# laughtervv/DISN

Hardware: AMD Instinct MI355X
Metric: SDF point queries/sec (137x137 img, 2048-pt batch, VGG-16 encode + two-stream query per batch) (higher is better)
Workload: dtype f32 results (products: two-term f16 split on v_mfma_f32_32x32x16_f16, ~22-bit operands, fp32 accumulate; gather / projection / resize / fc: fp32 FMA)

## Files before the change

### disn_amd/_lib.py

```python
from __future__ import annotations

import ctypes as C
import os
from typing import Optional

HERE = os.path.dirname(os.path.abspath(__file__))
LIB_PATH = os.environ.get("DISN_AMD_LIB") or os.path.join(HERE, "csrc", "libdisn_amd.so")
ABI_VERSION = 10

c_float_p = C.c_void_p


class DisnLibraryError(RuntimeError):
    pass


class DisnError(RuntimeError):
    def __init__(self, fn: str, status: int):
        kind = {-1: "invalid argument", -2: "unsupported shape", -3: "workspace too small",
                -4: "did not converge"}.get(
            status, "hipError_t %d" % status if status > 0 else "error")
        super().__init__("%s failed: %s (status %d)" % (fn, kind, status))
        self.status = status

# ... 51 lines not shown


I, Z, P, F, L = C.c_int, C.c_size_t, C.c_void_p, C.c_float, C.c_int64
SIGNATURES = {
    "disn_abi_version": (I, []),
    "disn_pack_kn": (I, [P, I, I, I, P, P]),
    "disn_pack_kn_x3_bytes": (Z, [I, I]),
    "disn_pack_kn_x3": (I, [P, I, I, P, P]),
    "disn_conv3x3_x3_workspace_bytes": (Z, [I, I, I, I, I]),
    "disn_conv3x3_x3": (I, [P, I, I, I, I, P, P, I, I, P, P, Z, P]),
    "disn_pack_conv_h2_bytes": (Z, [I, I]),
    "disn_pack_conv_h2": (I, [P, I, I, P, P]),
    "disn_conv_h2_gain_span": (I, [P, I, I, P, P]),
    "disn_conv1_1_workspace_bytes": (Z, []),
    "disn_conv1_1": (I, [P, I, I, I, P, P, I, P, P, P, Z, P]),
    "disn_conv3x3_h2_workspace_bytes": (Z, [I]),
    "disn_conv3x3_h2": (I, [P, I, I, I, I, P, P, I, I, P, P, P, I, P, Z, P]),
    "disn_conv3x3_h2_plan": (I, [I, I, I, I, I, I, P, P]),
    "disn_resize_bilinear": (I, [P, I, I, I, I, P, I, I, I, I, P]),
    "disn_vgg16_workspace_bytes": (Z, [I]),
    "disn_vgg16_forward": (I, [C.POINTER(VggWeights), P, I, P, C.POINTER(C.c_void_p * 5), P, P, Z, P]),
    "disn_vgg16_conv_stack": (I, [C.POINTER(VggWeights), P, I, P, C.POINTER(C.c_void_p * 5), P, P, Z, P]),
    "disn_conv3x3_workspace_bytes": (Z, [I, I, I, I, I]),
    "disn_conv3x3": (I, [P, I, I, I, I, P, P, I, I, P, P, Z, P]),
    "disn_conv3x3_planned_workspace_bytes": (Z, [I, I, I, I, I, I, I, I]),
    "disn_conv3x3_planned": (I, [P, I, I, I, I, P, P, I, I, P, P, Z, I, I, I, P]),
    "disn_maxpool2x2": (I, [P, I, I, I, I, P, P]),
    "disn_fc_workspace_bytes": (Z, [I, I, I]),
    "disn_fc": (I, [P, I, I, P, P, I, I, P, P, Z, P]),
    "disn_pack_dense_h2_bytes": (Z, [I, I]),
# ... 146 lines not shown
```

### disn_amd/csrc/api.hip

```cpp
#include "../../include/disn_amd.h"

#include "kernels.hpp"
#include "mesh_bvh.hpp"
#include "tuning.hpp"

#include <new>

using namespace disn;

#define DISN_TRY(expr)                    \
  do {                                    \
    hipError_t _e = (expr);               \
    if (_e != hipSuccess) return (int)_e; \
  } while (0)
#define DISN_RC(expr)        \
  do {                       \
    const int _rc = (expr);  \
    if (_rc) return _rc;     \
  } while (0)

namespace {

struct Bump {
  char* base;
// ... 522 lines not shown
  for (int i = 0; i < 3; ++i)
    if (!w->fc_w[i] || !w->fc_b[i]) return false;
  return true;
}

bool vgg_all_h2(const disn_vgg_weights_t* w) {
  for (int i = 0; i < 13; ++i)
    if (!w->conv_w_h2[i]) return false;
  return true;
}

int vgg_features(const disn_vgg_weights_t* w, const float* img, int B, float* resized,
                 float* const taps[5], float* featmap, const VggWs& s, const float** xio,
                 hipStream_t st, int i0 = 0, int i1 = 13) {
  const bool h2 = vgg_all_h2(w);
  if (i0 == 0)
    DISN_TRY(resize_bilinear_launch(img, B, DISN_IMG_H, DISN_IMG_W, 3, resized, DISN_VGG_SIZE,
                                    DISN_VGG_SIZE, 3, 0, st, 0, h2 ? s.amax : nullptr, h2 ? 14 * B * 64 : 0));
  const float* x = i0 == 0 ? resized : *xio;
  bool toggle = false;
  const size_t gws_cap = (size_t)((char*)s.fc_ws - (char*)s.gemm_ws);
  for (int i = 0; i < i1; ++i) {
    const VggLayer& L = kVgg[i];
    float* out = L.tap >= 0 ? taps[L.tap] : (L.hw >= 112 ? s.bufA : (toggle ? s.bufB : s.bufA));
    if (L.tap < 0 && L.hw < 112) toggle = !toggle;
    if (kPoolAfter[i]) toggle = false;
    if (i < i0) continue;
    bool pooled = false;
    if (h2 && i == 0) {
      DISN_TRY(conv1_1_direct_launch(x, B, L.hw, L.hw, static_cast<const float*>(w->conv_w_h2[0]), w->conv_b[0], 1, out,
                                     s.amax + (size_t)B * 64, st, 64));
    } else if (h2) {
      DISN_TRY(conv_h2_launch(x, B, L.hw, L.hw, L.cin, w->conv_w_h2[i], w->conv_b[i], L.cout, 1,
                              s.amax + (size_t)B * 64 * i, out, kPoolAfter[i] ? s.bufP : nullptr,
                              s.amax + (size_t)B * 64 * (i + 1), st, w->strict_forms == 1 ? kConvTilingStrict : kConvTilingAuto, 64));
      pooled = kPoolAfter[i];
    } else {
      DISN_RC(conv3x3_impl(x, B, L.hw, L.hw, L.cin, w->conv_w[i], w->conv_b[i], L.cout, 1, out, s.gemm_ws, gws_cap, st,
                           w->conv_w_x3[i], kPoolAfter[i] ? s.bufP : nullptr, &pooled));
    }
    x = out;
    if (L.tap >= 0 && featmap)
      DISN_TRY(resize_bilinear_launch(taps[L.tap], B, kTap[L.tap].hw, kTap[L.tap].hw, kTap[L.tap].ch,
                                      featmap, DISN_IMG_H, DISN_IMG_W, DISN_FEAT_DIM,
// ... 401 lines not shown
                      const float* pts_rot, int B, int N, float* resized224, float* const taps[5],
                      float* embedding, float* featmap, float* sdf, void* ws, size_t ws_bytes,
                      void* stream) {
  if (!ctx || !vgg_weights_ok(vw) || !mlp_weights_ok(mw) || !img || !trans_mat || !pts || !pts_rot ||
      !taps_ok(taps) || !embedding || !sdf || !ws || B <= 0 || N <= 0)
    return DISN_E_ARG;
  if ((long)B * N > kChunk || vw->num_classes != DISN_EMBED_DIM) return DISN_E_SHAPE;
  hipStream_t st = (hipStream_t)stream;
  const EncQueryWs e = encq_layout(ws, B, N, vw->num_classes);
  if (e.total > ws_bytes) return DISN_E_WS;
  float* resized = resized224 ? resized224 : e.vgg.resized;
  if (ctx->pipe_wait) DISN_TRY(hipStreamWaitEvent(st, ctx->pipe_wait, 0));
  const EncPlan p = encq_plan(vw, mw, B, N, featmap != nullptr);
  switch (p.form) {
    case ENC_FUSED_SMALL:
      return encq_fused_small(ctx, vw, mw, img, trans_mat, pts, pts_rot, B, N, resized, taps, embedding, sdf, e, st);
    case ENC_DENSE_H2:
      return encq_dense_h2(ctx, vw, mw, img, trans_mat, pts, pts_rot, B, N, resized, taps, embedding, featmap, sdf,
                           p.hb, p.strict, e, st);
    default:
      return encq_gemm_chain(ctx, vw, mw, img, trans_mat, pts, pts_rot, B, N, resized, taps, embedding, featmap, sdf,
                             e, st);
  }
}

int disn_build_featmap(const float* const taps[5], int B, float* featmap, void* stream) {
  if (!taps_ok(taps) || !featmap || B <= 0) return DISN_E_ARG;
  for (int i = 0; i < 5; ++i)
    DISN_TRY(resize_bilinear_launch(taps[i], B, kTap[i].hw, kTap[i].hw, kTap[i].ch, featmap, DISN_IMG_H,
                                    DISN_IMG_W, DISN_FEAT_DIM, kTap[i].off, (hipStream_t)stream));
  return 0;
// ... 643 lines not shown
```

### disn_amd/csrc/conv_h2.hip

```cpp
#include "kernels.hpp"
#include "tuning.hpp"
#include "h2_common.hpp"

#include <type_traits>

namespace disn {


__device__ __forceinline__ void h2_colmax_chunk(const float* __restrict__ p, long base, int mid, int inner,
                                                float* __restrict__ cmax_inner, float* __restrict__ cmax_mid,
                                                unsigned* tab_i, unsigned* tab_m) {
  const bool big_i = inner > 1024, big_m = mid > 1024;
  for (int i = threadIdx.x; i < 1024; i += 256) { tab_i[i] = 0u; tab_m[i] = 0u; }
  __syncthreads();
#pragma unroll
  for (int k = 0; k < 4; ++k) {
    const long e = base + (long)(k * 256 + threadIdx.x) * 4;
    const float4 v = *reinterpret_cast<const float4*>(p + e);
    const float a[4] = {fabsf(v.x), fabsf(v.y), fabsf(v.z), fabsf(v.w)};
    if (cmax_inner) {
      const int c0 = (int)(e % inner);
#pragma unroll
      for (int q = 0; q < 4; ++q) {
        if (big_i) atomicMax(reinterpret_cast<unsigned*>(cmax_inner) + c0 + q, __float_as_uint(a[q]));
// ... 466 lines not shown
    } else {
#pragma unroll
      for (int mb = 0; mb < MB; ++mb)
#pragma unroll
        for (int e = 0; e < NE; e += 2) {
          float m = fmaxf(val[mb][e], val[mb][e + 1]);
          m = fmaxf(m, __shfl_xor(m, 32));
          const int tx = (L0 & 15) + e0 + e, x = x0 + tx, y = y0 + 2 * mb;
          if (L0 < 16 && tx < TW && y + 1 < H && x + 1 < W) pb[((size_t)(y >> 1) * Wp + (x >> 1)) * Cout] = m;
        }
    }
  }
  CH2_STAMP(14);
}

template <int RT>
__global__ __launch_bounds__(256) void conv1_1_direct_kernel(const float* __restrict__ in, const float* __restrict__ w,
                                                             const float* __restrict__ bias, int B, int H, int W,
                                                             int relu, float* __restrict__ out,
                                                             float* __restrict__ out_amax, int amax_stride) {
  constexpr int PW = 40;
  constexpr int WR = 2 * RT + 2;
  constexpr int WE = WR * 34 * 3;
  constexpr int LQ = (WE + 255) / 256;
  __shared__ __attribute__((aligned(16))) float win[2][WR * 3 * PW];
  __shared__ __attribute__((aligned(16))) float wl[27 * 64];
  __shared__ float red[4];
  const int tid = threadIdx.x, c4 = tid & 15, pg = (tid >> 4) & 7, ry = tid >> 7;
  for (int i = tid; i < 27 * 16; i += 256)
    reinterpret_cast<float4*>(wl)[i] = reinterpret_cast<const float4*>(w)[i];
  __syncthreads();
  float4 wr[27];
#pragma unroll
  for (int k = 0; k < 27; ++k) wr[k] = *reinterpret_cast<const float4*>(&wl[k * 64 + 4 * c4]);
  const float4 bv = *reinterpret_cast<const float4*>(bias + 4 * c4);
  const int segs_x = (W + 31) >> 5, rows2 = (H + 2 * RT - 1) / (2 * RT);
  const long ntile = (long)B * rows2 * segs_x;
  float vmax = 0.f;
  int buf = 0, bcur = -1;
  auto flush = [&](int bimg) {
    float m = vmax;
#pragma unroll
// ... 21 lines not shown
    for (int k = 0; k < LQ; ++k) {
      const int i = tid + 256 * k;
      const int r = i / 102, rem = i - r * 102, px = rem / 3, c = rem - px * 3;
      const int yy = y0 - 1 + r, xx = x0 - 1 + px;
      v[k] = (i < WE && yy >= 0 && yy < H && xx >= 0 && xx < W) ? img[((size_t)yy * W + xx) * 3 + c] : 0.f;
    }
  };
  auto win_store = [&](int bf, const float (&v)[LQ]) {
#pragma unroll
    for (int k = 0; k < LQ; ++k) {
      const int i = tid + 256 * k;
      const int r = i / 102, rem = i - r * 102, px = rem / 3, c = rem - px * 3;
      if (i < WE) win[bf][(r * 3 + c) * PW + px] = v[k];
    }
  };
  float nxt[LQ];
  if ((long)blockIdx.x < ntile) {
    win_load(blockIdx.x, nxt);
    win_store(0, nxt);
  }
  __syncthreads();
  for (long tl = blockIdx.x; tl < ntile; tl += gridDim.x, buf ^= 1) {
    int b, y0, x0;
    tile_of(tl, b, y0, x0);
    if (out_amax && amax_stride && bcur >= 0 && b != bcur) flush(bcur);
    bcur = b;
    const bool more = tl + gridDim.x < ntile;
    if (more) win_load(tl + gridDim.x, nxt);
#pragma unroll 1
    for (int q = 0; q < RT; ++q) {
    float4 a[4] = {bv, bv, bv, bv};
#pragma unroll
    for (int r = 0; r < 3; ++r)
#pragma unroll
      for (int c = 0; c < 3; ++c) {
        const float* pl = &win[buf][((2 * q + ry + r) * 3 + c) * PW + 4 * pg];
        const float4 v0 = *reinterpret_cast<const float4*>(pl);
        const float2 v1 = *reinterpret_cast<const float2*>(pl + 4);
        const float v[6] = {v0.x, v0.y, v0.z, v0.w, v1.x, v1.y};
#pragma unroll
        for (int dx = 0; dx < 3; ++dx) {
          const float4 ww = wr[(r * 3 + dx) * 3 + c];
#pragma unroll
// ... 3 lines not shown
          }
        }
      }
    const int y = y0 + 2 * q + ry;
#pragma unroll
    for (int p = 0; p < 4; ++p) {
      float4 o = a[p];
      if (relu) { o.x = fmaxf(o.x, 0.f); o.y = fmaxf(o.y, 0.f); o.z = fmaxf(o.z, 0.f); o.w = fmaxf(o.w, 0.f); }
      const int x = x0 + 4 * pg + p;
      if (y < H && x < W) {
        *reinterpret_cast<float4*>(out + (((size_t)b * H + y) * W + x) * 64 + 4 * c4) = o;
        vmax = fmaxf(fmaxf(fmaxf(vmax, fabsf(o.x)), fabsf(o.y)), fmaxf(fabsf(o.z), fabsf(o.w)));
      }
    }
    }
    if (more) win_store(buf ^ 1, nxt);
    __syncthreads();
  }
  if (out_amax && bcur >= 0) flush(amax_stride ? bcur : 0);
}

hipError_t conv1_1_direct_launch(const float* in, int B, int H, int W, const float* w_hwio, const float* bias, int relu,
                                 float* out, float* out_amax, hipStream_t st, int amax_stride) {
  const int rt = B >= kConvWideMinImages ? 4 : 1;
  const long ntile = (long)B * ((H + 2 * rt - 1) / (2 * rt)) * ((W + 31) / 32);
  const int grid = (int)(ntile < 512 ? ntile : 512);
  if (rt == 4) hipLaunchKernelGGL(conv1_1_direct_kernel<4>, dim3(grid), dim3(256), 0, st, in, w_hwio, bias, B, H, W, relu, out, out_amax, amax_stride);
  else hipLaunchKernelGGL(conv1_1_direct_kernel<1>, dim3(grid), dim3(256), 0, st, in, w_hwio, bias, B, H, W, relu, out, out_amax, amax_stride);
  return hipGetLastError();
}

bool conv_h2_supported(int H, int W, int Cin, int Cout) {
  return Cin > 0 && Cin % 64 == 0 && Cout > 0 && Cout % 64 == 0 && H > 0 && W > 0 && H < 32768 && W < 32768 &&
         (size_t)H * W * (Cin > Cout ? Cin : Cout) < (size_t)1 << 31;
}

#ifndef CH2_UBENCH
namespace {
long form_grid(int form, int B, int H, int W, int Cout) {
  const ConvFormGeom& g = kConvForms[form];
  return (long)B * ((H + g.th - 1) / g.th) * ((W + g.tw - 1) / g.tw) * (Cout / g.nch);
}

// ... 191 lines not shown
size_t disn_conv1_1_workspace_bytes(void) { return 256; }

int disn_conv1_1(const float* in, int B, int H, int W, const float* w_hwio, const float* bias, int relu, float* out,
                 float* out_amax, void* ws, size_t ws_bytes, void* stream) {
  if (!in || !w_hwio || !bias || !out || !ws || B <= 0 || H <= 0 || W <= 0) return DISN_E_ARG;
  if (ws_bytes < 256) return DISN_E_WS;
  hipStream_t st = (hipStream_t)stream;
  float* slots = static_cast<float*>(ws);
  hipError_t e = hipSuccess;
  if (out_amax) e = hipMemsetAsync(slots, 0, 256, st);
  if (e == hipSuccess) e = disn::conv1_1_direct_launch(in, B, H, W, w_hwio, bias, relu, out, out_amax ? slots : nullptr, st);
  if (e == hipSuccess && out_amax) e = disn::amax_fold_launch(slots, out_amax, st);
  return e == hipSuccess ? 0 : (int)e;
}

}
#endif
```

### disn_amd/csrc/elementwise.hip

```cpp
#include "kernels.hpp"
#include "h2_common.hpp"

namespace disn {

#define DISN_FEAT 1472
#define DISN_FEAT4 368
#define DISN_IMG 137

template <int VEC>
__global__ __launch_bounds__(256) void resize_kernel(const float* __restrict__ in, int B, int Hin,
                                                     int Win, int C, float* __restrict__ out,
                                                     int Hout, int Wout, int out_cstride,
                                                     int out_coff, float sy, float sx,
                                                     float* __restrict__ zero, int nzero) {
  for (size_t i = (size_t)blockIdx.x * blockDim.x + threadIdx.x; i < (size_t)nzero; i += (size_t)gridDim.x * blockDim.x) zero[i] = 0.f;
  const int cv = C / VEC;
  const size_t total = (size_t)B * Hout * Wout * cv;
  for (size_t i = (size_t)blockIdx.x * blockDim.x + threadIdx.x; i < total;
       i += (size_t)gridDim.x * blockDim.x) {
    const int c = (int)(i % cv) * VEC;
    size_t pidx = i / cv;
    const int ox = (int)(pidx % Wout);
    pidx /= Wout;
    const int oy = (int)(pidx % Hout);
    const int b = (int)(pidx / Hout);
    const float fy = (float)oy * sy, fx = (float)ox * sx;
    const int ylo = (int)floorf(fy), xlo = (int)floorf(fx);
    const int yhi = min(ylo + 1, Hin - 1), xhi = min(xlo + 1, Win - 1);
    const float yl = fy - (float)ylo, xl = fx - (float)xlo;
    const float* base = in + (size_t)b * Hin * Win * C + c;
    const float* ptl = base + ((size_t)ylo * Win + xlo) * C;
    const float* ptr = base + ((size_t)ylo * Win + xhi) * C;
    const float* pbl = base + ((size_t)yhi * Win + xlo) * C;
    const float* pbr = base + ((size_t)yhi * Win + xhi) * C;
    float* po = out + ((size_t)(b * Hout + oy) * Wout + ox) * out_cstride + out_coff + c;
    if (VEC == 4) {
      const float4 tl = *reinterpret_cast<const float4*>(ptl);
      const float4 tr = *reinterpret_cast<const float4*>(ptr);
      const float4 bl = *reinterpret_cast<const float4*>(pbl);
      const float4 br = *reinterpret_cast<const float4*>(pbr);
      float4 o;
#define DISN_LERP(f)                              \
  {                                               \
    const float top = tl.f + (tr.f - tl.f) * xl;  \
    const float bot = bl.f + (br.f - bl.f) * xl;  \
    o.f = top + (bot - top) * yl;                 \
  }
      DISN_LERP(x) DISN_LERP(y) DISN_LERP(z) DISN_LERP(w)
#undef DISN_LERP
      *reinterpret_cast<float4*>(po) = o;
    } else {
      const float top = *ptl + (*ptr - *ptl) * xl;
      const float bot = *pbl + (*pbr - *pbl) * xl;
      *po = top + (bot - top) * yl;
    }
  }
}

static inline int grid_for(size_t total, int cap = 8192) {
  size_t b = (total + 255) / 256;
  if (b > (size_t)cap) b = cap;
  if (b < 1) b = 1;
  return (int)b;
}

hipError_t resize_bilinear_launch(const float* in, int B, int Hin, int Win, int C, float* out,
                                  int Hout, int Wout, int out_cstride, int out_coff,
                                  hipStream_t st, int max_blocks, float* zero, int nzero) {
  const int cap = max_blocks > 0 ? max_blocks : 8192;
// ... 742 lines not shown
```

### disn_amd/csrc/h2_common.hpp

```cpp
#pragma once
#include <hip/hip_runtime.h>

#include "kernels.hpp"

namespace disn {

typedef _Float16 ch_h8 __attribute__((ext_vector_type(8)));
typedef _Float16 ch_h4 __attribute__((ext_vector_type(4)));
typedef float ch_f16v __attribute__((ext_vector_type(16)));
typedef float ch_f2v __attribute__((ext_vector_type(2)));

namespace ch2 {
__host__ __device__ inline float pow2_scale(float amax, int target_exp) {
  union { float f; unsigned u; } a;
  a.f = amax;
  const int e = (int)((a.u >> 23) & 0xffu) - 127;
  if (!(amax > 0.f) || e > 100 || e < -100) return 1.0f;
  a.u = (unsigned)(127 + target_exp - e) << 23;
  return a.f;
}
__host__ __device__ constexpr int sigma(int i) {
  return i < 4 ? i : (i < 12 ? i + 12 : (i < 16 ? i - 8 : (i < 20 ? i + 8 : (i < 28 ? i - 12 : i))));
}
__host__ __device__ constexpr int quad_row(int q, int g) {
  return sigma(8 * q + 4 * g);
// ... 107 lines not shown
```

### disn_amd/csrc/kernels.hpp

```cpp
#pragma once
#include <hip/hip_runtime.h>
#include <stddef.h>
#include <stdint.h>

#include "../../include/disn_amd.h"

struct disn_ctx {
  hipStream_t aux;
  hipEvent_t ev[10];
  hipEvent_t pipe_wait = nullptr, pipe_record = nullptr;
};

namespace disn {

#ifdef __HIPCC__
typedef float nt_v4f __attribute__((ext_vector_type(4)));
__device__ __forceinline__ float4 nt_load4(const float* p) {
  const nt_v4f v = __builtin_nontemporal_load(reinterpret_cast<const nt_v4f*>(p));
  return make_float4(v[0], v[1], v[2], v[3]);
}
__device__ __forceinline__ void nt_store4(float* p, const float4& v) {
  nt_v4f t;
  t[0] = v.x; t[1] = v.y; t[2] = v.z; t[3] = v.w;
  __builtin_nontemporal_store(t, reinterpret_cast<nt_v4f*>(p));
// ... 295 lines not shown
  int form;
  int grid, block;
  int tiles_x, tiles_y;
};
ConvPlan conv_h2_plan(int B, int H, int W, int Cin, int Cout, int tiling);
hipError_t conv_h2_launch(const float* in, int B, int H, int W, int Cin, const void* wimg, const float* bias,
                          int Cout, int relu, const float* in_amax, float* out, float* pool_out, float* out_amax,
                          hipStream_t st, int tiling = kConvTilingAuto, int amax_stride = 0);

struct ConvH2Dev;
bool conv_h2w_supported(int H, int W, int Cin, int Cout);
hipError_t conv_h2w_launch(const ConvH2Dev& d, const ConvPlan& plan, hipStream_t st);

hipError_t conv1_1_direct_launch(const float* in, int B, int H, int W, const float* w_hwio, const float* bias, int relu,
                                 float* out, float* out_amax, hipStream_t st, int amax_stride = 0);

struct DenseH2Prob {
  const float* a;
  int lda;
  const float* a2;
  int lda2, k1;
  const float* in_bias;
  int in_bias_rows;
  const unsigned char* wimg;
  int Kimg;
  const float* bias;
  const float* in_amax;
  const float* in_amax2;
  int in_amax2_n;
  float* out;
// ... 57 lines not shown
```

### disn_amd/engine.py

```python
from __future__ import annotations

from dataclasses import dataclass
from typing import Dict, List, Optional

import time

import numpy as np
import torch

from . import ops
from ._lib import MLP_FIELDS, MlpWeights, VggWeights, lib
from .weights import MLP_SCOPES, VGG_CONV_NAMES, WeightStore


class DeviceWeights:

    def __init__(self, store: WeightStore, device: torch.device, conv_h2: bool = True, equalise: bool = True):
        if not store.complete():
            raise ValueError("WeightStore is incomplete")
        self.device = device
        self.num_classes = store.num_classes
        self._keep: List[torch.Tensor] = []
        dev = lambda a: self._hold(torch.from_numpy(np.ascontiguousarray(a, np.float32)).to(device))
        if equalise:
# ... 87 lines not shown
        for f in MLP_FIELDS:
            assert getattr(m, f), f
        self.mlp = m
        torch.cuda.current_stream(device).synchronize()

    def _hold(self, t: torch.Tensor) -> torch.Tensor:
        self._keep.append(t)
        return t


FOLD_MIN_POINTS = 32768


@dataclass
class Encoded:
    resized: torch.Tensor
    taps: List[torch.Tensor]
    embedding: torch.Tensor
    featmap: Optional[torch.Tensor]
    pred: Optional[torch.Tensor] = None
    pmap: Optional[dict] = None
    pmap_amax: Optional[dict] = None
    units: str = "true"


class SdfEngine:

    def __init__(self, store: Optional[WeightStore], device: Optional[torch.device] = None, fused: bool = True,
                 conv_h2: bool = True, weights: Optional[DeviceWeights] = None, equalise: bool = True,
                 strict: bool = False):
        if device is None:
# ... 71 lines not shown
        if enc.pmap is None:
            enc.pmap = {}
        if image_index not in enc.pmap:
            with torch.cuda.device(self.device):
                enc.pmap[image_index] = ops.fold_local(self.weights.mlp, self.featmap_of(enc)[image_index])
        return enc.pmap[image_index]

    def pmap_amax_of(self, enc: Encoded, image_index: int) -> torch.Tensor:
        if enc.pmap_amax is None:
            enc.pmap_amax = {}
        if image_index not in enc.pmap_amax:
            with torch.cuda.device(self.device):
                enc.pmap_amax[image_index] = ops.amax(self.pmap_of(enc, image_index))
        return enc.pmap_amax[image_index]

    def encode_query(self, imgs, pts, trans_mat, pts_rot=None, keep_featmap: bool = False):
        imgs, pts, trans_mat = self._dev(imgs), self._dev(pts), self._dev(trans_mat)
        pts_rot = pts if pts_rot is None else self._dev(pts_rot)
        with torch.cuda.device(self.device):
            ws = self._workspace("encq", lib().disn_encode_query_workspace_bytes(pts.shape[0], pts.shape[1]))
            resized, taps, emb, featmap, sdf = ops.encode_query(self._ctx, self._vgg, self.weights.mlp,
                                                                imgs, trans_mat, pts, pts_rot, ws, keep_featmap)
        return Encoded(resized, taps, emb, featmap, units=self._units()), sdf

    def query(self, enc: Encoded, pts, trans_mat, pts_rot=None, fold: Optional[bool] = None,
              fused: Optional[bool] = None) -> torch.Tensor:
        pts = self._dev(pts)
        pts_rot = pts if pts_rot is None else self._dev(pts_rot)
        trans_mat = self._dev(trans_mat)
        with torch.cuda.device(self.device):
            ws = self._workspace("query", lib().disn_query_workspace_bytes(pts.shape[0], pts.shape[1]))
            if fold is None:
                fold = pts.shape[1] >= FOLD_MIN_POINTS
            if fold:
                B = pts.shape[0]
                pm = self.pmap_of(enc, 0) if B == 1 else torch.stack([self.pmap_of(enc, b) for b in range(B)])
                if self.fused if fused is None else fused:
# ... 206 lines not shown
        self._dispatch(work, min(S, len(jobs)))
        for st in self.streams:
            cur.wait_stream(st)
        return out

    def run_calls(self, calls):
        S = len(self.engines)
        out = [None] * len(calls)
        cur = torch.cuda.current_stream(self.device)

        def work(i):
            if self.trace is not None:
                self.trace.append((i, "start", time.perf_counter()))
            self.streams[i].wait_stream(cur)
            for g in range(i, len(calls), S):
                out[g] = self.engines[i].encode_query(*calls[g])[1]
                if self.trace is not None:
                    self.trace.append((i, g, time.perf_counter()))

        self._dispatch(work, min(S, len(calls)))
        for st in self.streams:
            cur.wait_stream(st)
        return out

    @staticmethod
    def call_sizes(njobs: int, batch: int, in_flight: int, balance: bool):
        if njobs <= 0:
            return []
        n = -(-njobs // batch)
        if not balance:
            return [batch] * (njobs // batch) + ([njobs % batch] if njobs % batch else [])
# ... 33 lines not shown

        def check_one_shape(idx):
            if len({tuple(jobs[k][1].shape) for k in idx}) != 1:
                raise ValueError("jobs of one batch must have point sets of one shape")

        def work(i):
            if self.trace is not None:
                self.trace.append((i, "start", time.perf_counter()))
            self.streams[i].wait_stream(cur)
            for g in mine[i]:
                idx = groups[g]
                check_one_shape(idx)
                args = [cat(idx, p) for p in range(len(jobs[idx[0]]))]
                if self.trace is not None:
                    self.trace.append((i, "call %d" % g, time.perf_counter()))
                enc, sdf = self.engines[i].encode_query(*args)
                if self.trace is not None:
                    self.trace.append((i, g, time.perf_counter()))
                o = 0
                for k in idx:
                    b = jobs[k][0].shape[0]
                    if keep_encoded:
                        e = Encoded(enc.resized[o:o + b], [t[o:o + b] for t in enc.taps], enc.embedding[o:o + b], None, units=enc.units)
                        out[k] = (e, sdf[o:o + b])
                    else:
                        out[k] = sdf[o:o + b]
                    o += b

        if chained and len(groups) > 1:
            with torch.cuda.device(self.device):
                if not hasattr(self, "_conv_done"):
                    self._conv_done = [torch.cuda.Event() for _ in range(S + 1)]
                    for e in self._conv_done:
                        e.record()
                for st in self.streams:
                    st.wait_stream(cur)
                prev = None
                try:
                    for g, idx in enumerate(groups):
                        i = g % S
                        check_one_shape(idx)
                        rec = self._conv_done[g % (S + 1)]
                        ops.ctx_pipeline(self.engines[i]._ctx, prev, rec)
                        with torch.cuda.stream(self.streams[i]):
                            args = [cat(idx, p) for p in range(len(jobs[idx[0]]))]
                            enc, sdf = self.engines[i].encode_query(*args)
                        o = 0
                        for k in idx:
                            b = jobs[k][0].shape[0]
                            out[k] = (Encoded(enc.resized[o:o + b], [t[o:o + b] for t in enc.taps], enc.embedding[o:o + b], None, units=enc.units),
                                      sdf[o:o + b]) if keep_encoded else sdf[o:o + b]
                            o += b
                        prev = rec
                finally:
                    for eng in self.engines:
                        ops.ctx_pipeline(eng._ctx, None, None)
            for st in self.streams:
                cur.wait_stream(st)
            return out
        self._dispatch(work, min(S, len(groups)))
        for st in self.streams:
# ... 3 lines not shown
```

### disn_amd/ops.py

```python
from __future__ import annotations

import ctypes as C
from typing import List, Optional, Sequence, Tuple

import numpy as np
import torch

from . import _lib
from ._lib import MlpWeights, VggWeights, check, lib

FEAT_DIM = 1472
IMG = 137
TAP_SHAPES = ((224, 64), (112, 128), (56, 256), (28, 512), (14, 512))


def _stream() -> int:
    return torch.cuda.current_stream().cuda_stream


def _chk(t: torch.Tensor, name: str) -> torch.Tensor:
    if not (isinstance(t, torch.Tensor) and t.is_cuda and t.dtype == torch.float32):
        raise TypeError("%s must be a float32 CUDA tensor (the HIP path has no CPU fallback)" % name)
    return t if t.is_contiguous() else t.contiguous()

# ... 91 lines not shown

def conv1_1(x: torch.Tensor, w_hwio: torch.Tensor, bias: torch.Tensor, relu: bool = True, want_amax: bool = False):
    x, w = _chk(x, "x"), _chk(w_hwio, "w_hwio")
    B, H, W, Cin = x.shape
    if Cin != 3 or w.numel() != 27 * 64:
        raise ValueError("conv1_1: expected 3 -> 64 channels")
    out = torch.empty((B, H, W, 64), dtype=torch.float32, device=x.device)
    amax = torch.zeros(1, dtype=torch.float32, device=x.device) if want_amax else None
    ws = _ws(lib().disn_conv1_1_workspace_bytes(), x.device)
    check("disn_conv1_1", lib().disn_conv1_1(x.data_ptr(), B, H, W, w.data_ptr(), bias.data_ptr(), int(relu),
                                             out.data_ptr(), amax.data_ptr() if want_amax else None, ws.data_ptr(),
                                             ws.numel(), _stream()))
    return (out, amax) if want_amax else out


def pack_conv_h2(w_hwio: torch.Tensor) -> torch.Tensor:
    w = _chk(w_hwio, "w_hwio")
    cout = w.shape[-1]
    cin = w.numel() // (9 * cout)
    nbytes = lib().disn_pack_conv_h2_bytes(cin, cout)
    if nbytes == 0:
        raise ValueError("pack_conv_h2: Cin and Cout must be multiples of 64, got %d, %d" % (cin, cout))
    out = torch.empty(nbytes, dtype=torch.uint8, device=w.device)
    check("disn_pack_conv_h2", lib().disn_pack_conv_h2(w.data_ptr(), cin, cout, out.data_ptr(), _stream()))
    return out


def conv_h2_gain_span(image: torch.Tensor, cin: int, cout: int):
    span = C.c_float(0.0)
    rc = lib().disn_conv_h2_gain_span(image.data_ptr(), int(cin), int(cout), C.byref(span), _stream())
# ... 155 lines not shown
    h = C.c_void_p()
    check("disn_ctx_create", lib().disn_ctx_create(C.byref(h)))
    return h.value


def ctx_pipeline(ctx: int, wait_event: Optional[torch.cuda.Event], record_event: Optional[torch.cuda.Event]) -> None:
    check("disn_ctx_pipeline", lib().disn_ctx_pipeline(ctx, wait_event.cuda_event if wait_event is not None else None,
                                                       record_event.cuda_event if record_event is not None else None))


def ctx_destroy(ctx: int) -> None:
    if ctx:
        check("disn_ctx_destroy", lib().disn_ctx_destroy(ctx))


def _alloc_encoder_outputs(B: int, num_classes: int, dev, featmap: bool = True):
    resized = torch.empty((B, 224, 224, 3), dtype=torch.float32, device=dev)
    taps = [torch.empty((B, hw, hw, ch), dtype=torch.float32, device=dev) for hw, ch in TAP_SHAPES]
    emb = torch.empty((B, num_classes), dtype=torch.float32, device=dev)
    fm = torch.empty((B, IMG, IMG, FEAT_DIM), dtype=torch.float32, device=dev) if featmap else None
    return resized, taps, emb, fm


def encode(ctx: Optional[int], w: VggWeights, img: torch.Tensor, ws: Optional[torch.Tensor] = None):
    img = _chk_img(img)
    B = img.shape[0]
    resized, taps, emb, featmap = _alloc_encoder_outputs(B, w.num_classes, img.device)
    ws = _fit_ws(ws, lib().disn_encode_workspace_bytes(B), img.device)
    tp = _tap_ptrs(taps, chk=False)
    check("disn_encode", lib().disn_encode(ctx, C.byref(w), img.data_ptr(), B, resized.data_ptr(), C.byref(tp),
                                           emb.data_ptr(), featmap.data_ptr(), ws.data_ptr(), ws.numel(), _stream()))
    return resized, taps, emb, featmap


def encode_query(ctx: int, vw: VggWeights, mw: MlpWeights, img: torch.Tensor, trans_mat: torch.Tensor,
                 pts: torch.Tensor, pts_rot: Optional[torch.Tensor] = None, ws: Optional[torch.Tensor] = None,
                 keep_featmap: bool = True):
    img, pts, trans_mat = _chk(img, "img"), _chk(pts, "pts"), _chk(trans_mat, "trans_mat")
    pts_rot = pts if pts_rot is None else _chk(pts_rot, "pts_rot")
    B, N = pts.shape[0], pts.shape[1]
    resized, taps, emb, featmap = _alloc_encoder_outputs(B, vw.num_classes, img.device, keep_featmap)
    sdf = torch.empty((B, N), dtype=torch.float32, device=img.device)
    need = lib().disn_encode_query_workspace_bytes(B, N)
    if need == 0:
        raise ValueError("encode_query needs B*N <= 65536")
    ws = _fit_ws(ws, need, img.device)
    tp = _tap_ptrs(taps, chk=False)
    check("disn_encode_query", lib().disn_encode_query(
        ctx, C.byref(vw), C.byref(mw), img.data_ptr(), trans_mat.data_ptr(), pts.data_ptr(), pts_rot.data_ptr(),
        B, N, resized.data_ptr(), C.byref(tp), emb.data_ptr(), featmap.data_ptr() if keep_featmap else None,
        sdf.data_ptr(), ws.data_ptr(), ws.numel(), _stream()))
    return resized, taps, emb, featmap, sdf


def build_featmap(taps: Sequence[torch.Tensor], out: Optional[torch.Tensor] = None) -> torch.Tensor:
    B = taps[0].shape[0]
    if out is None:
        out = torch.empty((B, IMG, IMG, FEAT_DIM), dtype=torch.float32, device=taps[0].device)
    tp = _tap_ptrs(taps)
    check("disn_build_featmap", lib().disn_build_featmap(C.byref(tp), B, out.data_ptr(), _stream()))
    return out


def project(pts: torch.Tensor, trans_mat: torch.Tensor) -> torch.Tensor:
    pts, trans_mat = _chk(pts, "pts"), _chk(trans_mat, "trans_mat")
# ... 482 lines not shown
```

### include/disn_amd.h

```cpp
#ifndef DISN_AMD_H
#define DISN_AMD_H

#include <stddef.h>
#include <stdint.h>

#ifdef __cplusplus
extern "C" {
#endif

#define DISN_IMG_H 137
#define DISN_IMG_W 137
#define DISN_VGG_SIZE 224
#define DISN_FEAT_DIM 1472
#define DISN_EMBED_DIM 1024

#define DISN_E_ARG (-1)
#define DISN_E_SHAPE (-2)
#define DISN_E_WS (-3)
#define DISN_E_CONVERGE (-4)

#define DISN_ABI_VERSION 10
int disn_abi_version(void);

int disn_pack_kn(const float* w_kn, int K, int N, int Kpad, float* packed, void* stream);
size_t disn_pack_kn_x3_bytes(int K, int N);
int disn_pack_kn_x3(const float* w_kn, int K, int N, void* packed, void* stream);
size_t disn_conv3x3_x3_workspace_bytes(int B, int H, int W, int Cin, int Cout);
int disn_conv3x3_x3(const float* in, int B, int H, int W, int Cin, const void* w_x3, const float* bias,
                    int Cout, int relu, float* out, void* ws, size_t ws_bytes, void* stream);
size_t disn_pack_conv_h2_bytes(int Cin, int Cout);
int disn_pack_conv_h2(const float* w_hwio, int Cin, int Cout, void* image, void* stream);
#define DISN_W_GAIN_SPAN 1
int disn_conv_h2_gain_span(const void* image, int Cin, int Cout, float* span_log2, void* stream);
size_t disn_conv1_1_workspace_bytes(void);
int disn_conv1_1(const float* in, int B, int H, int W, const float* w_hwio, const float* bias, int relu, float* out,
                 float* out_amax, void* ws, size_t ws_bytes, void* stream);
size_t disn_conv3x3_h2_workspace_bytes(int B);
int disn_conv3x3_h2(const float* in, int B, int H, int W, int Cin, const void* image, const float* bias, int Cout,
                    int relu, float* out, float* pool_out, float* out_amax, int tiling, void* ws, size_t ws_bytes,
                    void* stream);
int disn_conv3x3_h2_plan(int B, int H, int W, int Cin, int Cout, int tiling, int* grid, int* block);

int disn_resize_bilinear(const float* in, int B, int Hin, int Win, int C, float* out, int Hout,
                         int Wout, int out_cstride, int out_coff, void* stream);

typedef struct disn_vgg_weights {
  const float* conv_w[13];
  const float* conv_b[13];
  const float* fc_w[3];
  const float* fc_b[3];
  int num_classes;
// ... 314 lines not shown
```

Before: 17.19 million.

## Fuse bilinear resize of input image into conv1_1 direct kernel

Adds a template variant of the conv1_1 direct kernel that loads the 137x137 source tile into shared memory and bilinearly resamples it on the fly into the conv window. This removes the separate resize kernel and the 224x224x3 intermediate write and read when the caller does not keep the resized image. A two-deep prefetch pipeline for source tiles is added, and the amax slots are zeroed with a memset. The pipeline entry points now pass keep_resized=False. This costs extra shared memory and resampling arithmetic inside conv1_1.

After: 17.09 million. About the same (-0.6%).

```diff
diff --git a/disn_amd/_lib.py b/disn_amd/_lib.py
--- a/disn_amd/_lib.py
+++ b/disn_amd/_lib.py
@@ -89,6 +89,7 @@
     "disn_conv_h2_gain_span": (I, [P, I, I, P, P]),
     "disn_conv1_1_workspace_bytes": (Z, []),
     "disn_conv1_1": (I, [P, I, I, I, P, P, I, P, P, P, Z, P]),
+    "disn_conv1_1_resized": (I, [P, I, I, I, I, I, P, P, I, I, P, P, P, P]),
     "disn_conv3x3_h2_workspace_bytes": (Z, [I]),
     "disn_conv3x3_h2": (I, [P, I, I, I, I, P, P, I, I, P, P, P, I, P, Z, P]),
     "disn_conv3x3_h2_plan": (I, [I, I, I, I, I, I, P, P]),
diff --git a/disn_amd/csrc/api.hip b/disn_amd/csrc/api.hip
--- a/disn_amd/csrc/api.hip
+++ b/disn_amd/csrc/api.hip
@@ -560,9 +560,11 @@
                  float* const taps[5], float* featmap, const VggWs& s, const float** xio,
                  hipStream_t st, int i0 = 0, int i1 = 13) {
   const bool h2 = vgg_all_h2(w);
-  if (i0 == 0)
+  if (!resized && !h2) return DISN_E_ARG;
+  if (i0 == 0 && resized)
     DISN_TRY(resize_bilinear_launch(img, B, DISN_IMG_H, DISN_IMG_W, 3, resized, DISN_VGG_SIZE,
                                     DISN_VGG_SIZE, 3, 0, st, 0, h2 ? s.amax : nullptr, h2 ? 14 * B * 64 : 0));
+  if (i0 == 0 && !resized) DISN_TRY(hipMemsetAsync(s.amax, 0, (size_t)14 * B * 64 * sizeof(float), st));
   const float* x = i0 == 0 ? resized : *xio;
   bool toggle = false;
   const size_t gws_cap = (size_t)((char*)s.fc_ws - (char*)s.gemm_ws);
@@ -573,7 +575,10 @@
     if (kPoolAfter[i]) toggle = false;
     if (i < i0) continue;
     bool pooled = false;
-    if (h2 && i == 0) {
+    if (h2 && i == 0 && !resized) {
+      DISN_TRY(conv1_1_resize_launch(img, B, DISN_IMG_H, DISN_IMG_W, L.hw, L.hw, static_cast<const float*>(w->conv_w_h2[0]),
+                                     w->conv_b[0], 1, out, s.amax + (size_t)B * 64, st, 64));
+    } else if (h2 && i == 0) {
       DISN_TRY(conv1_1_direct_launch(x, B, L.hw, L.hw, static_cast<const float*>(w->conv_w_h2[0]), w->conv_b[0], 1, out,
                                      s.amax + (size_t)B * 64, st, 64));
     } else if (h2) {
@@ -1005,7 +1010,7 @@
   const EncPlan p = encq_plan(vw, mw, B, N, featmap != nullptr);
   switch (p.form) {
     case ENC_FUSED_SMALL:
-      return encq_fused_small(ctx, vw, mw, img, trans_mat, pts, pts_rot, B, N, resized, taps, embedding, sdf, e, st);
+      return encq_fused_small(ctx, vw, mw, img, trans_mat, pts, pts_rot, B, N, resized224, taps, embedding, sdf, e, st);
     case ENC_DENSE_H2:
       return encq_dense_h2(ctx, vw, mw, img, trans_mat, pts, pts_rot, B, N, resized, taps, embedding, featmap, sdf,
                            p.hb, p.strict, e, st);
diff --git a/disn_amd/csrc/conv_h2.hip b/disn_amd/csrc/conv_h2.hip
--- a/disn_amd/csrc/conv_h2.hip
+++ b/disn_amd/csrc/conv_h2.hip
@@ -504,11 +504,14 @@
   CH2_STAMP(14);
 }
 
-template <int RT>
+constexpr int conv1_1_src_rows(int rt) { return ((2 * rt + 2) * 5) / 8 + 2; }
+constexpr int kConv1SrcCols = (34 * 5) / 8 + 2;
+template <int RT, bool RS>
 __global__ __launch_bounds__(256) void conv1_1_direct_kernel(const float* __restrict__ in, const float* __restrict__ w,
                                                              const float* __restrict__ bias, int B, int H, int W,
                                                              int relu, float* __restrict__ out,
-                                                             float* __restrict__ out_amax, int amax_stride) {
+                                                             float* __restrict__ out_amax, int amax_stride,
+                                                             int Hs, int Ws, float sy, float sx) {
   constexpr int PW = 40;
   constexpr int WR = 2 * RT + 2;
   constexpr int WE = WR * 34 * 3;
@@ -516,6 +519,10 @@
   __shared__ __attribute__((aligned(16))) float win[2][WR * 3 * PW];
   __shared__ __attribute__((aligned(16))) float wl[27 * 64];
   __shared__ float red[4];
+  constexpr int SR = conv1_1_src_rows(RT), SC = kConv1SrcCols;
+  constexpr int SE = SR * SC * 3;
+  constexpr int LS = (SE + 255) / 256;
+  __shared__ float stage[RS ? 2 : 1][RS ? SE : 1];
   const int tid = threadIdx.x, c4 = tid & 15, pg = (tid >> 4) & 7, ry = tid >> 7;
   for (int i = tid; i < 27 * 16; i += 256)
     reinterpret_cast<float4*>(wl)[i] = reinterpret_cast<const float4*>(w)[i];
@@ -567,8 +574,63 @@
       if (i < WE) win[bf][(r * 3 + c) * PW + px] = v[k];
     }
   };
-  float nxt[LQ];
-  if ((long)blockIdx.x < ntile) {
+  auto src_origin = [&](int y0, int x0, int& ys0, int& xs0) {
+    int hi;
+    float fr;
+    resize_coord(max(y0 - 1, 0), sy, Hs, ys0, hi, fr);
+    resize_coord(max(x0 - 1, 0), sx, Ws, xs0, hi, fr);
+  };
+  auto src_load = [&](long tl, float (&v)[LS]) {
+    int b, y0, x0, ys0, xs0;
+    tile_of(tl, b, y0, x0);
+    src_origin(y0, x0, ys0, xs0);
+    const float* img = in + (size_t)b * Hs * Ws * 3;
+#pragma unroll
+    for (int k = 0; k < LS; ++k) {
+      const int i = tid + 256 * k;
+      const int r = i / (SC * 3), yy = ys0 + r, xo = xs0 * 3 + (i - r * SC * 3);
+      v[k] = (i < SE && yy < Hs && xo < Ws * 3) ? img[(size_t)yy * Ws * 3 + xo] : 0.f;
+    }
+  };
+  auto stage_store = [&](int sg, const float (&v)[LS]) {
+#pragma unroll
+    for (int k = 0; k < LS; ++k)
+      if (tid + 256 * k < SE) stage[sg][tid + 256 * k] = v[k];
+  };
+  auto win_resample = [&](int bf, int sg, long tl) {
+    int b, y0, x0, ys0, xs0;
+    tile_of(tl, b, y0, x0);
+    src_origin(y0, x0, ys0, xs0);
+#pragma unroll
+    for (int k = 0; k < LQ; ++k) {
+      const int i = tid + 256 * k;
+      const int r = i / 102, rem = i - r * 102, px = rem / 3, c = rem - px * 3;
+      const int yy = y0 - 1 + r, xx = x0 - 1 + px;
+      float v = 0.f;
+      if (i < WE && yy >= 0 && yy < H && xx >= 0 && xx < W) {
+        int ylo, yhi, xlo, xhi;
+        float yl, xl;
+        resize_coord(yy, sy, Hs, ylo, yhi, yl);
+        resize_coord(xx, sx, Ws, xlo, xhi, xl);
+        const float* s0 = &stage[sg][((ylo - ys0) * SC + (xlo - xs0)) * 3 + c];
+        const int dx = (xhi - xlo) * 3, dy = (yhi - ylo) * SC * 3;
+        v = resize_lerp(s0[0], s0[dx], s0[dy], s0[dy + dx], xl, yl);
+      }
+      if (i < WE) win[bf][(r * 3 + c) * PW + px] = v;
+    }
+  };
+  float nxt[RS ? LS : LQ];
+  if constexpr (RS) {
+    const bool one = (long)blockIdx.x < ntile, two = (long)blockIdx.x + gridDim.x < ntile;
+    if (one) {
+      src_load(blockIdx.x, nxt);
+      stage_store(0, nxt);
+    }
+    if (two) src_load((long)blockIdx.x + gridDim.x, nxt);
+    __syncthreads();
+    if (one) win_resample(0, 0, blockIdx.x);
+    if (two) stage_store(1, nxt);
+  } else if ((long)blockIdx.x < ntile) {
     win_load(blockIdx.x, nxt);
     win_store(0, nxt);
   }
@@ -579,7 +641,13 @@
     if (out_amax && amax_stride && bcur >= 0 && b != bcur) flush(bcur);
     bcur = b;
     const bool more = tl + gridDim.x < ntile;
-    if (more) win_load(tl + gridDim.x, nxt);
+    const bool more2 = RS && tl + 2 * (long)gridDim.x < ntile;
+    if constexpr (RS) {
+      if (more2) src_load(tl + 2 * (long)gridDim.x, nxt);
+      if (more) win_resample(buf ^ 1, buf ^ 1, tl + gridDim.x);
+    } else if (more) {
+      win_load(tl + gridDim.x, nxt);
+    }
 #pragma unroll 1
     for (int q = 0; q < RT; ++q) {
     float4 a[4] = {bv, bv, bv, bv};
@@ -613,7 +681,11 @@
       }
     }
     }
-    if (more) win_store(buf ^ 1, nxt);
+    if constexpr (RS) {
+      if (more2) stage_store(buf, nxt);
+    } else if (more) {
+      win_store(buf ^ 1, nxt);
+    }
     __syncthreads();
   }
   if (out_amax && bcur >= 0) flush(amax_stride ? bcur : 0);
@@ -624,8 +696,36 @@
   const int rt = B >= kConvWideMinImages ? 4 : 1;
   const long ntile = (long)B * ((H + 2 * rt - 1) / (2 * rt)) * ((W + 31) / 32);
   const int grid = (int)(ntile < 512 ? ntile : 512);
-  if (rt == 4) hipLaunchKernelGGL(conv1_1_direct_kernel<4>, dim3(grid), dim3(256), 0, st, in, w_hwio, bias, B, H, W, relu, out, out_amax, amax_stride);
-  else hipLaunchKernelGGL(conv1_1_direct_kernel<1>, dim3(grid), dim3(256), 0, st, in, w_hwio, bias, B, H, W, relu, out, out_amax, amax_stride);
+  if (rt == 4) hipLaunchKernelGGL((conv1_1_direct_kernel<4, false>), dim3(grid), dim3(256), 0, st, in, w_hwio, bias, B, H, W, relu, out, out_amax, amax_stride, 0, 0, 0.f, 0.f);
+  else hipLaunchKernelGGL((conv1_1_direct_kernel<1, false>), dim3(grid), dim3(256), 0, st, in, w_hwio, bias, B, H, W, relu, out, out_amax, amax_stride, 0, 0, 0.f, 0.f);
+  return hipGetLastError();
+}
+
+static bool conv1_1_src_fits(int n_out, int n_in, int step, int wlen, int cap) {
+  const float s = (float)n_in / (float)n_out;
+  if ((int)floorf((float)(n_out - 1) * s) > n_in - 1) return false;
+  for (int o0 = 0; o0 < n_out; o0 += step) {
+    const int a = o0 > 0 ? o0 - 1 : 0, b = o0 - 2 + wlen < n_out - 1 ? o0 - 2 + wlen : n_out - 1;
+    const int lo = (int)floorf((float)a * s), hi1 = (int)floorf((float)b * s) + 1;
+    if ((hi1 < n_in - 1 ? hi1 : n_in - 1) - lo + 1 > cap) return false;
+  }
+  return true;
+}
+bool conv1_1_resize_supported(int B, int Hs, int Ws, int H, int W) {
+  const int rt = B >= kConvWideMinImages ? 4 : 1;
+  return Hs > 0 && Ws > 0 && H > 0 && W > 0 &&
+         conv1_1_src_fits(H, Hs, 2 * rt, 2 * rt + 2, rt == 4 ? conv1_1_src_rows(4) : conv1_1_src_rows(1)) &&
+         conv1_1_src_fits(W, Ws, 32, 34, kConv1SrcCols);
+}
+hipError_t conv1_1_resize_launch(const float* src, int B, int Hs, int Ws, int H, int W, const float* w_hwio,
+                                 const float* bias, int relu, float* out, float* out_amax, hipStream_t st, int amax_stride) {
+  if (!conv1_1_resize_supported(B, Hs, Ws, H, W)) return hipErrorInvalidValue;
+  const int rt = B >= kConvWideMinImages ? 4 : 1;
+  const long ntile = (long)B * ((H + 2 * rt - 1) / (2 * rt)) * ((W + 31) / 32);
+  const int grid = (int)(ntile < 512 ? ntile : 512);
+  const float sy = (float)Hs / (float)H, sx = (float)Ws / (float)W;
+  if (rt == 4) hipLaunchKernelGGL((conv1_1_direct_kernel<4, true>), dim3(grid), dim3(256), 0, st, src, w_hwio, bias, B, H, W, relu, out, out_amax, amax_stride, Hs, Ws, sy, sx);
+  else hipLaunchKernelGGL((conv1_1_direct_kernel<1, true>), dim3(grid), dim3(256), 0, st, src, w_hwio, bias, B, H, W, relu, out, out_amax, amax_stride, Hs, Ws, sy, sx);
   return hipGetLastError();
 }
 
@@ -847,5 +947,22 @@
   return e == hipSuccess ? 0 : (int)e;
 }
 
+int disn_conv1_1_resized(const float* src, int B, int Hs, int Ws, int H, int W, const float* w_hwio, const float* bias,
+                         int relu, int fused, float* resized, float* out, float* slots, void* stream) {
+  if (!src || !w_hwio || !bias || !out || !slots || (!fused && !resized) || B <= 0 || Hs <= 0 || Ws <= 0 || H <= 0 || W <= 0)
+    return DISN_E_ARG;
+  hipStream_t st = (hipStream_t)stream;
+  hipError_t e;
+  if (fused) {
+    if (!disn::conv1_1_resize_supported(B, Hs, Ws, H, W)) return DISN_E_SHAPE;
+    e = hipMemsetAsync(slots, 0, (size_t)B * 64 * sizeof(float), st);
+    if (e == hipSuccess) e = disn::conv1_1_resize_launch(src, B, Hs, Ws, H, W, w_hwio, bias, relu, out, slots, st, 64);
+  } else {
+    e = disn::resize_bilinear_launch(src, B, Hs, Ws, 3, resized, H, W, 3, 0, st, 0, slots, B * 64);
+    if (e == hipSuccess) e = disn::conv1_1_direct_launch(resized, B, H, W, w_hwio, bias, relu, out, slots, st, 64);
+  }
+  return e == hipSuccess ? 0 : (int)e;
+}
+
 }
 #endif
diff --git a/disn_amd/csrc/elementwise.hip b/disn_amd/csrc/elementwise.hip
--- a/disn_amd/csrc/elementwise.hip
+++ b/disn_amd/csrc/elementwise.hip
@@ -24,10 +24,10 @@
     pidx /= Wout;
     const int oy = (int)(pidx % Hout);
     const int b = (int)(pidx / Hout);
-    const float fy = (float)oy * sy, fx = (float)ox * sx;
-    const int ylo = (int)floorf(fy), xlo = (int)floorf(fx);
-    const int yhi = min(ylo + 1, Hin - 1), xhi = min(xlo + 1, Win - 1);
-    const float yl = fy - (float)ylo, xl = fx - (float)xlo;
+    int ylo, yhi, xlo, xhi;
+    float yl, xl;
+    resize_coord(oy, sy, Hin, ylo, yhi, yl);
+    resize_coord(ox, sx, Win, xlo, xhi, xl);
     const float* base = in + (size_t)b * Hin * Win * C + c;
     const float* ptl = base + ((size_t)ylo * Win + xlo) * C;
     const float* ptr = base + ((size_t)ylo * Win + xhi) * C;
@@ -40,19 +40,13 @@
       const float4 bl = *reinterpret_cast<const float4*>(pbl);
       const float4 br = *reinterpret_cast<const float4*>(pbr);
       float4 o;
-#define DISN_LERP(f)                              \
-  {                                               \
-    const float top = tl.f + (tr.f - tl.f) * xl;  \
-    const float bot = bl.f + (br.f - bl.f) * xl;  \
-    o.f = top + (bot - top) * yl;                 \
-  }
-      DISN_LERP(x) DISN_LERP(y) DISN_LERP(z) DISN_LERP(w)
-#undef DISN_LERP
+      o.x = resize_lerp(tl.x, tr.x, bl.x, br.x, xl, yl);
+      o.y = resize_lerp(tl.y, tr.y, bl.y, br.y, xl, yl);
+      o.z = resize_lerp(tl.z, tr.z, bl.z, br.z, xl, yl);
+      o.w = resize_lerp(tl.w, tr.w, bl.w, br.w, xl, yl);
       *reinterpret_cast<float4*>(po) = o;
     } else {
-      const float top = *ptl + (*ptr - *ptl) * xl;
-      const float bot = *pbl + (*pbr - *pbl) * xl;
-      *po = top + (bot - top) * yl;
+      *po = resize_lerp(*ptl, *ptr, *pbl, *pbr, xl, yl);
     }
   }
 }
diff --git a/disn_amd/csrc/h2_common.hpp b/disn_amd/csrc/h2_common.hpp
--- a/disn_amd/csrc/h2_common.hpp
+++ b/disn_amd/csrc/h2_common.hpp
@@ -9,6 +9,22 @@
 typedef _Float16 ch_h4 __attribute__((ext_vector_type(4)));
 typedef float ch_f16v __attribute__((ext_vector_type(16)));
 typedef float ch_f2v __attribute__((ext_vector_type(2)));
+
+#ifdef __HIPCC__
+__device__ __forceinline__ void resize_coord(int o, float scale, int n_in, int& lo, int& hi, float& frac) {
+#pragma clang fp contract(off)
+  const float f = (float)o * scale;
+  lo = (int)floorf(f);
+  hi = min(lo + 1, n_in - 1);
+  frac = f - (float)lo;
+}
+__device__ __forceinline__ float resize_lerp(float tl, float tr, float bl, float br, float xl, float yl) {
+#pragma clang fp contract(off)
+  const float top = tl + (tr - tl) * xl;
+  const float bot = bl + (br - bl) * xl;
+  return top + (bot - top) * yl;
+}
+#endif
 
 namespace ch2 {
 __host__ __device__ inline float pow2_scale(float amax, int target_exp) {
diff --git a/disn_amd/csrc/kernels.hpp b/disn_amd/csrc/kernels.hpp
--- a/disn_amd/csrc/kernels.hpp
+++ b/disn_amd/csrc/kernels.hpp
@@ -333,6 +333,9 @@
 
 hipError_t conv1_1_direct_launch(const float* in, int B, int H, int W, const float* w_hwio, const float* bias, int relu,
                                  float* out, float* out_amax, hipStream_t st, int amax_stride = 0);
+bool conv1_1_resize_supported(int B, int Hs, int Ws, int H, int W);
+hipError_t conv1_1_resize_launch(const float* src, int B, int Hs, int Ws, int H, int W, const float* w_hwio,
+                                 const float* bias, int relu, float* out, float* out_amax, hipStream_t st, int amax_stride = 0);
 
 struct DenseH2Prob {
   const float* a;
diff --git a/disn_amd/engine.py b/disn_amd/engine.py
--- a/disn_amd/engine.py
+++ b/disn_amd/engine.py
@@ -125,7 +125,7 @@
 
 @dataclass
 class Encoded:
-    resized: torch.Tensor
+    resized: Optional[torch.Tensor]
     taps: List[torch.Tensor]
     embedding: torch.Tensor
     featmap: Optional[torch.Tensor]
@@ -227,13 +227,14 @@
                 enc.pmap_amax[image_index] = ops.amax(self.pmap_of(enc, image_index))
         return enc.pmap_amax[image_index]
 
-    def encode_query(self, imgs, pts, trans_mat, pts_rot=None, keep_featmap: bool = False):
+    def encode_query(self, imgs, pts, trans_mat, pts_rot=None, keep_featmap: bool = False, keep_resized: bool = True):
         imgs, pts, trans_mat = self._dev(imgs), self._dev(pts), self._dev(trans_mat)
         pts_rot = pts if pts_rot is None else self._dev(pts_rot)
         with torch.cuda.device(self.device):
             ws = self._workspace("encq", lib().disn_encode_query_workspace_bytes(pts.shape[0], pts.shape[1]))
             resized, taps, emb, featmap, sdf = ops.encode_query(self._ctx, self._vgg, self.weights.mlp,
-                                                                imgs, trans_mat, pts, pts_rot, ws, keep_featmap)
+                                                                imgs, trans_mat, pts, pts_rot, ws, keep_featmap,
+                                                                keep_resized)
         return Encoded(resized, taps, emb, featmap, units=self._units()), sdf
 
     def query(self, enc: Encoded, pts, trans_mat, pts_rot=None, fold: Optional[bool] = None,
@@ -470,7 +471,7 @@
                 self.trace.append((i, "start", time.perf_counter()))
             self.streams[i].wait_stream(cur)
             for g in range(i, len(calls), S):
-                out[g] = self.engines[i].encode_query(*calls[g])[1]
+                out[g] = self.engines[i].encode_query(*calls[g], keep_resized=False)[1]
                 if self.trace is not None:
                     self.trace.append((i, g, time.perf_counter()))
 
@@ -534,7 +535,7 @@
                 args = [cat(idx, p) for p in range(len(jobs[idx[0]]))]
                 if self.trace is not None:
                     self.trace.append((i, "call %d" % g, time.perf_counter()))
-                enc, sdf = self.engines[i].encode_query(*args)
+                enc, sdf = self.engines[i].encode_query(*args, keep_resized=keep_encoded)
                 if self.trace is not None:
                     self.trace.append((i, g, time.perf_counter()))
                 o = 0
@@ -564,7 +565,7 @@
                         ops.ctx_pipeline(self.engines[i]._ctx, prev, rec)
                         with torch.cuda.stream(self.streams[i]):
                             args = [cat(idx, p) for p in range(len(jobs[idx[0]]))]
-                            enc, sdf = self.engines[i].encode_query(*args)
+                            enc, sdf = self.engines[i].encode_query(*args, keep_resized=keep_encoded)
                         o = 0
                         for k in idx:
                             b = jobs[k][0].shape[0]
diff --git a/disn_amd/ops.py b/disn_amd/ops.py
--- a/disn_amd/ops.py
+++ b/disn_amd/ops.py
@@ -129,6 +129,21 @@
     return (out, amax) if want_amax else out
 
 
+def conv1_1_resized(src: torch.Tensor, w_hwio: torch.Tensor, bias: torch.Tensor, size: int = 224, fused: bool = True,
+                    relu: bool = True):
+    src, w = _chk(src, "src"), _chk(w_hwio, "w_hwio")
+    B, Hs, Ws, Cin = src.shape
+    if Cin != 3 or w.numel() != 27 * 64:
+        raise ValueError("conv1_1: expected 3 -> 64 channels")
+    out = torch.empty((B, size, size, 64), dtype=torch.float32, device=src.device)
+    slots = torch.empty((B, 64), dtype=torch.float32, device=src.device)
+    resized = None if fused else torch.empty((B, size, size, 3), dtype=torch.float32, device=src.device)
+    check("disn_conv1_1_resized", lib().disn_conv1_1_resized(
+        src.data_ptr(), B, Hs, Ws, size, size, w.data_ptr(), bias.data_ptr(), int(relu), int(fused),
+        None if fused else resized.data_ptr(), out.data_ptr(), slots.data_ptr(), _stream()))
+    return out, slots, resized
+
+
 def pack_conv_h2(w_hwio: torch.Tensor) -> torch.Tensor:
     w = _chk(w_hwio, "w_hwio")
     cout = w.shape[-1]
@@ -314,8 +329,8 @@
         check("disn_ctx_destroy", lib().disn_ctx_destroy(ctx))
 
 
-def _alloc_encoder_outputs(B: int, num_classes: int, dev, featmap: bool = True):
-    resized = torch.empty((B, 224, 224, 3), dtype=torch.float32, device=dev)
+def _alloc_encoder_outputs(B: int, num_classes: int, dev, featmap: bool = True, resized: bool = True):
+    resized = torch.empty((B, 224, 224, 3), dtype=torch.float32, device=dev) if resized else None
     taps = [torch.empty((B, hw, hw, ch), dtype=torch.float32, device=dev) for hw, ch in TAP_SHAPES]
     emb = torch.empty((B, num_classes), dtype=torch.float32, device=dev)
     fm = torch.empty((B, IMG, IMG, FEAT_DIM), dtype=torch.float32, device=dev) if featmap else None
@@ -335,11 +350,11 @@
 
 def encode_query(ctx: int, vw: VggWeights, mw: MlpWeights, img: torch.Tensor, trans_mat: torch.Tensor,
                  pts: torch.Tensor, pts_rot: Optional[torch.Tensor] = None, ws: Optional[torch.Tensor] = None,
-                 keep_featmap: bool = True):
+                 keep_featmap: bool = True, keep_resized: bool = True):
     img, pts, trans_mat = _chk(img, "img"), _chk(pts, "pts"), _chk(trans_mat, "trans_mat")
     pts_rot = pts if pts_rot is None else _chk(pts_rot, "pts_rot")
     B, N = pts.shape[0], pts.shape[1]
-    resized, taps, emb, featmap = _alloc_encoder_outputs(B, vw.num_classes, img.device, keep_featmap)
+    resized, taps, emb, featmap = _alloc_encoder_outputs(B, vw.num_classes, img.device, keep_featmap, keep_resized)
     sdf = torch.empty((B, N), dtype=torch.float32, device=img.device)
     need = lib().disn_encode_query_workspace_bytes(B, N)
     if need == 0:
@@ -348,7 +363,7 @@
     tp = _tap_ptrs(taps, chk=False)
     check("disn_encode_query", lib().disn_encode_query(
         ctx, C.byref(vw), C.byref(mw), img.data_ptr(), trans_mat.data_ptr(), pts.data_ptr(), pts_rot.data_ptr(),
-        B, N, resized.data_ptr(), C.byref(tp), emb.data_ptr(), featmap.data_ptr() if keep_featmap else None,
+        B, N, resized.data_ptr() if keep_resized else None, C.byref(tp), emb.data_ptr(), featmap.data_ptr() if keep_featmap else None,
         sdf.data_ptr(), ws.data_ptr(), ws.numel(), _stream()))
     return resized, taps, emb, featmap, sdf
 
diff --git a/include/disn_amd.h b/include/disn_amd.h
--- a/include/disn_amd.h
+++ b/include/disn_amd.h
@@ -35,6 +35,8 @@
 size_t disn_conv1_1_workspace_bytes(void);
 int disn_conv1_1(const float* in, int B, int H, int W, const float* w_hwio, const float* bias, int relu, float* out,
                  float* out_amax, void* ws, size_t ws_bytes, void* stream);
+int disn_conv1_1_resized(const float* src, int B, int Hs, int Ws, int H, int W, const float* w_hwio, const float* bias,
+                         int relu, int fused, float* resized, float* out, float* slots, void* stream);
 size_t disn_conv3x3_h2_workspace_bytes(int B);
 int disn_conv3x3_h2(const float* in, int B, int H, int W, int Cin, const void* image, const float* bias, int Cout,
                     int relu, float* out, float* pool_out, float* out_amax, int tiling, void* ws, size_t ws_bytes,
```
